# david8862/tf-keras-speech-commands

Measured on AMD Instinct MI355X. Metric: 1 s@16 kHz clips/sec train-step, simple_cnn bs4096, 1/2/4/8 MI355X; eval top-1, higher is better.
Workload: dtype f32; 1 GPU; configs[1]: simple_cnn train step = featurize(f32 1 s @16 kHz) + fwd + bwd + Adam, 36 logits (background + 35 words), batch 4096 per GPU; global_batch=4096, parallelism=dp1, gradient_exchange=none (one rank), rccl_ranks=0, library_build=546ca62dfe01

## Files before the change

### tf-keras-speech-commands_amd/csrc/kws_conv.h

```cpp
#pragma once
#include "kws_device.h"

namespace kws {

struct ConvGeom {
    int B, H, W, Ho, Wo;
    int stride, pt, pl;
    int KH, KW;
    int pmajor = 0;
};

enum { EPI_NONE = 0, EPI_RELU = 1, EPI_BIAS_RELU6 = 2, EPI_BIAS = 3, EPI_BIAS_RELU = 4,
       EPI_BN_RELU6 = 5,
       EPI_BNBWD_GATE6 = 6 };
enum { MODE_FWD = 0, MODE_DGRAD = 1 };

__host__ __device__ constexpr int stride16(int c) { return (c % 32 == 16) ? c : c + 16; }

template <int CR, int CO, int MODE, int EPI>
__global__ __launch_bounds__(256) void conv_gemm_kernel(const float *__restrict__ src, const float *__restrict__ wgt,
                                                         const float *__restrict__ bias, float *__restrict__ dst,
                                                         ConvGeom g)
{
    constexpr int KC = CR >= 32 ? 32 : CR;
// ... 570 lines not shown
        __syncthreads();
#pragma unroll
        for (int mt = 0; mt < MT; ++mt)
#pragma unroll
            for (int nw = 0; nw < NW; ++nw)
#pragma unroll
                for (int r = 0; r < 4; ++r) red[(16 * mt + 4 * lq + r) * COUT + 16 * (wave * NW + nw) + li] = acc[t][mt][nw][r];
        __syncthreads();
        if (nchunks > 0)
            for (int i = tid; i < CIN * COUT; i += 256) atomicAdd(dw + (long)(tap0 + t) * CIN * COUT + i, red[i]);
    }
}

template <int N>
__device__ __forceinline__ void load_vec(const float *__restrict__ p, float (&v)[N])
{
    if constexpr (N == 1) {
        v[0] = p[0];
    } else if constexpr (N == 2) {
        const float2 t = *reinterpret_cast<const float2 *>(p);
        v[0] = t.x; v[1] = t.y;
    } else {
#pragma unroll
        for (int i = 0; i < N / 4; ++i) {
            const float4 t = *reinterpret_cast<const float4 *>(p + 4 * i);
            v[4 * i] = t.x; v[4 * i + 1] = t.y; v[4 * i + 2] = t.z; v[4 * i + 3] = t.w;
        }
    }
}

template <int CIN, int COUT, int GPB>
__global__ __launch_bounds__(256) void conv_wgrad_direct_kernel(const float *__restrict__ x, const float *__restrict__ dz,
                                                                 float *__restrict__ dw, const float *__restrict__ zeros,
                                                                 ConvGeom g, int steps_per_wave)
{
    constexpr int CB = CIN >= 64 ? 64 : CIN;
    constexpr int CBLK = CIN / CB;
    constexpr int MT = CB / 16, NT = COUT / 16;
    static_assert(CIN % CB == 0 && CB % 16 == 0 && COUT % 16 == 0, "channel counts must be multiples of 16");
    extern __shared__ __attribute__((aligned(16))) float red[];

    const int lane = threadIdx.x & 63, wave = threadIdx.x >> 6, li = lane & 15, lq = lane >> 4;
    const long M = (long)g.B * g.Ho * g.Wo;
    const int HoWo = g.Ho * g.Wo;
    const int ngroups = g.KH * g.KW * CBLK, grp0 = blockIdx.y * GPB;
    const long step0 = ((long)blockIdx.x * 4 + wave) * steps_per_wave;

    int kh[GPB], kw[GPB], cb[GPB], toff[GPB];
    bool gok[GPB];
#pragma unroll
    for (int gi = 0; gi < GPB; ++gi) {
        const int grp = grp0 + gi, tap = grp / CBLK;
        gok[gi] = grp < ngroups;
        kh[gi] = tap / g.KW;
        kw[gi] = tap % g.KW;
        cb[gi] = (grp % CBLK) * CB;
        toff[gi] = (kh[gi] * g.W + kw[gi]) * CIN + cb[gi];
    }

    f32x4 acc[GPB][MT][NT];
#pragma unroll
    for (int gi = 0; gi < GPB; ++gi)
#pragma unroll
        for (int mt = 0; mt < MT; ++mt)
#pragma unroll
            for (int nt = 0; nt < NT; ++nt) acc[gi][mt][nt] = (f32x4){0.f, 0.f, 0.f, 0.f};

    long p = step0 * 4 + lq;
    int b = (int)(p / HoWo), rem = (int)(p % HoWo), oh = rem / g.Wo, ow = rem % g.Wo;
    auto load_frags = [&](float (&af)[GPB][MT], float (&bf)[NT]) {
        const bool pok = p < M;
        load_vec<NT>(pok ? dz + ((int)p * COUT + NT * li) : zeros + NT * li, bf);
        const int y0 = oh * g.stride - g.pt, x0 = ow * g.stride - g.pl;
// ... 982 lines not shown
```

### tf-keras-speech-commands_amd/csrc/kws_device.h

```cpp
#pragma once
#include <hip/hip_runtime.h>
#include <stdint.h>

namespace kws {

typedef float f32x4 __attribute__((ext_vector_type(4)));


__device__ __forceinline__ f32x4 mfma16(float a, float b, f32x4 c)
{
    return __builtin_amdgcn_mfma_f32_16x16x4f32(a, b, c, 0, 0, 0);
}

typedef __bf16 bf16x8 __attribute__((ext_vector_type(8)));
typedef __bf16 bf16x4 __attribute__((ext_vector_type(4)));
__device__ __forceinline__ f32x4 mfma_bf16(bf16x8 a, bf16x8 b, f32x4 c)
{
    return __builtin_amdgcn_mfma_f32_16x16x32_bf16(a, b, c, 0, 0, 0);
}
__device__ __forceinline__ f32x4 mfma_bf16x6(const bf16x8 (&a)[3], const bf16x8 (&b)[3], f32x4 c)
{
    c = mfma_bf16(a[1], b[1], c);
    c = mfma_bf16(a[2], b[0], c);
    c = mfma_bf16(a[0], b[2], c);
// ... 49 lines not shown
    return __int_as_float(__builtin_amdgcn_readlane(__float_as_int(v), 63));
}
#undef KWS_DPP_ADD

struct HeadFwdArgs {
    const float *b2;
    const int32_t *labels;
    const float *class_w;
    float *probs, *loss_i_out, *correct_i_out;
    float grad_scale;
    int ignore_index;
};

constexpr int kAccSlots = 8, kAccDoubles = kAccSlots * 2 * 128;
__device__ __forceinline__ void acc_add(double *__restrict__ acc, int C2, int i, double v)
{
    atomicAdd(acc + (blockIdx.x & (kAccSlots - 1)) * C2 + i, v);
}
__device__ __forceinline__ double acc_sum(const double *__restrict__ acc, int C2, int i)
{
    double v[kAccSlots];
#pragma unroll
    for (int j = 0; j < kAccSlots; ++j) v[j] = acc[j * C2 + i];
    double t = 0.0;
#pragma unroll
    for (int j = 0; j < kAccSlots; ++j) t += v[j];
    return t;
}
__device__ __forceinline__ void acc_clear(double *__restrict__ acc, int tid, int nthreads)
{
    for (int i = tid; i < kAccDoubles; i += nthreads) acc[i] = 0.0;
}

}
```

### tf-keras-speech-commands_amd/csrc/kws_layers.h

```cpp
#pragma once
#include "kws_device.h"

namespace kws {

constexpr float kBnEps = 1e-3f;
constexpr double kBnMomentum = 0.99;
constexpr float kCeEps = 1e-7f;
constexpr int kStatStride = 1024;

__device__ __forceinline__ double block_sum_partials(const double *__restrict__ partial, int which, int C, int c, int nblk,
                                                     double *sh )
{
    double s = 0.0;
    for (int b = threadIdx.x; b < nblk; b += 256) s += partial[((long)which * C + c) * kStatStride + b];
    sh[threadIdx.x] = s;
    __syncthreads();
    for (int o = 128; o > 0; o >>= 1) {
        if ((int)threadIdx.x < o) sh[threadIdx.x] += sh[threadIdx.x + o];
        __syncthreads();
    }
    s = sh[0];
    __syncthreads();
    return s;
}
// ... 449 lines not shown
    f32x4 d;
#pragma unroll
    for (int e = 0; e < 4; ++e) {
        const int c = c0 + e;
        const float xhat = (zv[e] - k.mean[c]) * k.inv[c];
        float v = gamma[c] * k.inv[c] * (gv[e] - k.k2[c] - xhat * k.k3[c]);
        if (RELU_IN) v = zv[e] > 0.f ? v : 0.f;
        d[e] = v;
    }
    bf16x4 h, m, l;
    split_bf16(d, h, m, l);
    reinterpret_cast<bf16x4 *>(out.p[0])[i4] = h;
    reinterpret_cast<bf16x4 *>(out.p[1])[i4] = m;
    reinterpret_cast<bf16x4 *>(out.p[2])[i4] = l;
}

struct BnAccBwd { const double *acc; double *acc_clear_set; long M; float *dgamma, *dbeta; };
__device__ __forceinline__ void bn_bwd_k_prologue(const BnAccBwd &a, const BnCoef &k, int C, float *kk)
{
    const int i = threadIdx.x;
    if (i < 2 * C) {
        const double t = acc_sum(a.acc, 2 * C, i);
        const float kv = (float)(t / (double)a.M);
        kk[i] = kv;
        if (blockIdx.x == 0) {
            if (i < C) { a.dbeta[i] = (float)t; k.k2[i] = kv; }
            else { a.dgamma[i - C] = (float)t; k.k3[i - C] = kv; }
        }
    }
    if (blockIdx.x == 0 && a.acc_clear_set) acc_clear(a.acc_clear_set, threadIdx.x, blockDim.x);
    __syncthreads();
}

template <bool RELU_IN>
__global__ __launch_bounds__(256) void bn_bwd_apply_routed_planes_kernel(const float *__restrict__ z, const float *__restrict__ gq,
                                                                          const unsigned char *__restrict__ arg, BnCoef k,
                                                                          const float *__restrict__ gamma, int B, int H, int W, int C,
                                                                          BnAccBwd a, Bf16PlanesOut out)
{
    __shared__ float kk[256];
    bn_bwd_k_prologue(a, k, C, kk);
    const int Hp = H / 2, Wp = W / 2, C4 = C / 4;
    const long total4 = (long)B * H * W * C4;
    for (long i4 = (long)blockIdx.x * 256 + threadIdx.x; i4 < total4; i4 += (long)gridDim.x * 256) {
        const int c0 = (int)(i4 % C4) * 4;
        const long pix = i4 / C4;
        const int p = (int)(pix % ((long)H * W)), b = (int)(pix / ((long)H * W)), y = p / W, x = p - y * W, ph = y >> 1, pw = x >> 1;
        const f32x4 zv = reinterpret_cast<const f32x4 *>(z)[i4];
        f32x4 gv = {0.f, 0.f, 0.f, 0.f};
        if (ph < Hp && pw < Wp) {
            const long q = (((long)b * Hp + ph) * Wp + pw) * C + c0;
            const f32x4 g4 = *reinterpret_cast<const f32x4 *>(gq + q);
            const unsigned a4 = *reinterpret_cast<const unsigned *>(arg + q), e = (unsigned)((y & 1) * 2 + (x & 1));
#pragma unroll
            for (int j = 0; j < 4; ++j) gv[j] = ((a4 >> (8 * j)) & 0xffu) == e ? g4[j] : 0.f;
        }
        f32x4 d;
#pragma unroll
        for (int j = 0; j < 4; ++j) {
            const int c = c0 + j;
            const float xhat = (zv[j] - k.mean[c]) * k.inv[c];
            float v = gamma[c] * k.inv[c] * (gv[j] - kk[c] - xhat * kk[C + c]);
            if (RELU_IN) v = zv[j] > 0.f ? v : 0.f;
            d[j] = v;
        }
        bf16x4 h, m, l;
        split_bf16(d, h, m, l);
        reinterpret_cast<bf16x4 *>(out.p[0])[i4] = h;
        reinterpret_cast<bf16x4 *>(out.p[1])[i4] = m;
        reinterpret_cast<bf16x4 *>(out.p[2])[i4] = l;
    }
}

template <bool RELU_IN>
__global__ __launch_bounds__(256) void bn_bwd_apply_acc_kernel(const float *__restrict__ z, float *__restrict__ gz, BnCoef k,
                                                                const float *__restrict__ gamma, long total4, int C, BnAccBwd a)
{
    __shared__ float kk[256];
    bn_bwd_k_prologue(a, k, C, kk);
    const int C4 = C / 4;
    for (long i4 = (long)blockIdx.x * 256 + threadIdx.x; i4 < total4; i4 += (long)gridDim.x * 256) {
        const int c0 = (int)(i4 % C4) * 4;
        const f32x4 zv = reinterpret_cast<const f32x4 *>(z)[i4], gv = reinterpret_cast<const f32x4 *>(gz)[i4];
        f32x4 d;
#pragma unroll
        for (int j = 0; j < 4; ++j) {
            const int c = c0 + j;
            const float xhat = (zv[j] - k.mean[c]) * k.inv[c];
            float v = gamma[c] * k.inv[c] * (gv[j] - kk[c] - xhat * kk[C + c]);
            if (RELU_IN) v = zv[j] > 0.f ? v : 0.f;
            d[j] = v;
        }
        reinterpret_cast<f32x4 *>(gz)[i4] = d;
    }
}

__global__ __launch_bounds__(256) void head_fwd_kernel(const float *__restrict__ d1, const float *__restrict__ w2,
                                                        const float *__restrict__ b2, const int32_t *__restrict__ labels,
                                                        const float *__restrict__ class_w, float *__restrict__ probs,
                                                        int32_t *__restrict__ argmax_out, float *__restrict__ loss_i,
                                                        float *__restrict__ correct_i, float *__restrict__ dlogits, int B,
                                                        int K, int C, float grad_scale, int ignore_index)
{
    extern __shared__ float hs[];
    float *xs = hs;
    float *lg = hs + 16 * K;
    const int b0 = blockIdx.x * 16;
    for (int i = threadIdx.x; i < 16 * K; i += 256) {
        const int s = i / K;
        xs[i] = (b0 + s < B) ? d1[(long)(b0 + s) * K + (i % K)] : 0.f;
    }
    __syncthreads();
    for (int i = threadIdx.x; i < 16 * C; i += 256) {
        const int s = i / C, c = i % C;
        float acc = 0.f;
        for (int k = 0; k < K; ++k) acc = fmaf(xs[s * K + k], w2[(long)k * C + c], acc);
        lg[i] = acc + b2[c];
    }
    __syncthreads();
    if (threadIdx.x < 16 && b0 + threadIdx.x < B) {
        const int s = threadIdx.x, b = b0 + s;
        float mx = lg[s * C];
        int am = 0;
        for (int c = 1; c < C; ++c)
            if (lg[s * C + c] > mx) { mx = lg[s * C + c]; am = c; }
        float sum = 0.f;
// ... 63 lines not shown
        if (omx > mx || (omx == mx && oam < am)) { mx = omx; am = oam; }
    }
    float sum = 0.f;
    for (int c = j; c < C; c += 16) { const float e = expf(lg[s * C + c] - mx); lg[s * C + c] = e; sum += e; }
#pragma unroll
    for (int o = 8; o > 0; o >>= 1) sum += __shfl_xor(sum, o, 16);
    const float rs = 1.f / sum;
    if (b >= B) return;
    if (argmax_out && j == 0) argmax_out[b] = am;
    if (probs)
        for (int c = j; c < C; c += 16) probs[(long)b * C + c] = lg[s * C + c] * rs;
    if (labels) {
        const int y = labels[b];
        const float py = lg[s * C + y] * rs;
        float loss, coef;
        if (class_w) {
            loss = -logf(py) * class_w[y];
            coef = class_w[y];
        } else {
            const float lo = kCeEps, hi = 1.f - kCeEps;
            loss = -logf(fminf(fmaxf(py, lo), hi));
            coef = (py >= lo && py <= hi) ? 1.f : 0.f;
        }
        if (ignore_index > 0 && y == ignore_index) { loss = 0.f; coef = 0.f; }
        if (j == 0) { loss_i[b] = loss; correct_i[b] = am == y ? 1.f : 0.f; }
        if (dlogits)
            for (int c = j; c < C; c += 16) dlogits[(long)b * C + c] = (lg[s * C + c] * rs - (c == y ? 1.f : 0.f)) * coef * grad_scale;
    }
}

__global__ __launch_bounds__(256) void loss_reduce_kernel(const float *__restrict__ loss_i, const float *__restrict__ correct_i,
                                                           int B, float *__restrict__ out)
{
    double s = 0.0, c = 0.0;
    for (int i = threadIdx.x; i < B; i += 256) { s += (double)loss_i[i]; c += (double)correct_i[i]; }
    __shared__ double sh[2][256];
    sh[0][threadIdx.x] = s;
    sh[1][threadIdx.x] = c;
    __syncthreads();
    for (int o = 128; o > 0; o >>= 1) {
        if (threadIdx.x < o) { sh[0][threadIdx.x] += sh[0][threadIdx.x + o]; sh[1][threadIdx.x] += sh[1][threadIdx.x + o]; }
        __syncthreads();
    }
    if (threadIdx.x == 0) { out[0] = (float)sh[0][0]; out[1] = (float)sh[1][0]; }
}

constexpr int kHeadBwdRows = 16;

template <bool RELU6_GATE>
__global__ __launch_bounds__(256) void head_bwd_kernel(const float *__restrict__ x, const float *__restrict__ w2,
                                                        const float *__restrict__ dlogits, float *__restrict__ dx,
                                                        float *__restrict__ dw2, float *__restrict__ db2, int B, int K, int C)
{
    extern __shared__ float hs[];
    float *xs = hs;
    float *ds = hs + kHeadBwdRows * K;
    const int b0 = blockIdx.x * kHeadBwdRows;
    for (int i = threadIdx.x; i < kHeadBwdRows * K; i += 256) xs[i] = (b0 + i / K < B) ? x[(long)(b0 + i / K) * K + (i % K)] : 0.f;
    for (int i = threadIdx.x; i < kHeadBwdRows * C; i += 256) ds[i] = (b0 + i / C < B) ? dlogits[(long)(b0 + i / C) * C + (i % C)] : 0.f;
    __syncthreads();
    for (int i = threadIdx.x; i < kHeadBwdRows * K; i += 256) {
        const int s = i / K, k = i % K;
        if (b0 + s >= B) continue;
        float acc = 0.f;
        for (int c = 0; c < C; ++c) acc = fmaf(ds[s * C + c], w2[(long)k * C + c], acc);
        if (RELU6_GATE) { const float xv = xs[i]; acc = (xv > 0.f && xv < 6.f) ? acc : 0.f; }
        dx[(long)(b0 + s) * K + k] = acc;
    }
    for (int i = threadIdx.x; i < K * C; i += 256) {
        const int k = i / C, c = i % C;
        float acc = 0.f;
        for (int s = 0; s < kHeadBwdRows; ++s) acc = fmaf(xs[s * K + k], ds[s * C + c], acc);
        if (dw2) atomicAdd(dw2 + i, acc);
    }
    for (int c = threadIdx.x; c < C; c += 256) {
        float acc = 0.f;
        for (int s = 0; s < kHeadBwdRows; ++s) acc += ds[s * C + c];
// ... 267 lines not shown
```

### tf-keras-speech-commands_amd/csrc/kws_model.hip

```cpp
#include <cstdlib>
#include <cstring>
#include <string>
#include <type_traits>
#include <vector>

#include "kws_common.h"
#include "kws_model_types.h"
#include "kws_conv.h"
#include "kws_layers.h"
#include "kws_layer1.h"
#include "kws_layer1_moments.h"
#include "kws_layer1_fast.h"
#include "kws_l1_conv2.h"
#include "kws_conv2_wgrad_fast.h"
#include "kws_lite.h"
#include "kws_lite_f16.h"
#include "kws_infer_fused.h"
#include "kws_conv_group.h"
#include "kws_dense_head.h"
#include "kws_cnn_plan.h"

using namespace kws;

namespace {
// ... 131 lines not shown
    KWS_LAUNCH("bn_infer_coef_all_kernel", bn_infer_coef_all_kernel, dim3(4), dim3(128), 0, s, a);
    return KWS_OK;
}

inline void stat_grid(long M, int C, int &nblk, int &rows)
{
    const int R = 256 / C;
    long want = (M + (long)R * 8 - 1) / ((long)R * 8);
    nblk = (int)std::min<long>(kMaxStatBlocks, std::max<long>(1, want));
    rows = (int)((M + nblk - 1) / nblk);
    nblk = (int)((M + rows - 1) / rows);
}

template <int CR, int CO, int MODE, int EPI>
int launch_gemm(const float *src, const float *w, const float *bias, float *dst, const ConvGeom &g, hipStream_t s)
{
    const long M = (long)g.B * g.Ho * g.Wo;
    static const std::string name = std::string("conv_gemm_fwd<") + std::to_string(CR) + "," +
                                    std::to_string(CO) + ">";
    KWS_LAUNCH(name.c_str(), (conv_gemm_kernel<CR, CO, MODE, EPI>), dim3(blocks_for(M, 64)), dim3(256), 0, s, src, w, bias, dst, g);
    return KWS_OK;
}

static int cu_count() { return device_cus(); }
template <typename K>
static int resident_blocks(K kernel, int threads, size_t smem)
{
    int nb = 0;
    if (hipOccupancyMaxActiveBlocksPerMultiprocessor(&nb, kernel, threads, smem) != hipSuccess || nb < 1) { (void)hipGetLastError(); nb = 1; }
    return nb;
}

template <int CIN, int COUT, int GPB>
int launch_wgrad(const float *x, const float *dz, float *dw, const ConvGeom &g, hipStream_t s, bool deterministic = false)
{
    const float *zp = zero_page();
    if (!zp) return fail(KWS_ERR_NOMEM, "cannot allocate the zero page on this device");
    constexpr int CB = CIN >= 64 ? 64 : CIN;
    constexpr size_t smem = (4 * 64 * 4 + 16 * COUT) * sizeof(float);
    const long M = (long)g.B * g.Ho * g.Wo;
    const int ngroups = g.KH * g.KW * (CIN / CB), gy = (ngroups + GPB - 1) / GPB;
    const long steps = (M + 3) / 4;
    static const int occ = resident_blocks(conv_wgrad_direct_kernel<CIN, COUT, GPB>, 256, smem);
    const long slots = deterministic ? 1 : std::max<long>(1, (long)cu_count() * occ / gy);
    const long gx_want = std::max<long>(1, std::min<long>(slots, (steps + 4 * 8 - 1) / (4 * 8)));
    const int spw = (int)((steps + 4 * gx_want - 1) / (4 * gx_want));
    const long gx = (steps + 4L * spw - 1) / (4L * spw);
    static const std::string name = "conv_wgrad<" + std::to_string(CIN) + "," + std::to_string(COUT) + ">";
    KWS_LAUNCH(name.c_str(), (conv_wgrad_direct_kernel<CIN, COUT, GPB>), dim3((unsigned)gx, (unsigned)gy), dim3(256), smem,
               s, x, dz, dw, zp, g, spw);
    return KWS_OK;
}

template <int CIN, int COUT, int TPB, bool DPRE = false, bool XBN = false>
int launch_wgrad_bf16(const float *x, const float *dz, float *dw, const ConvGeom &g, hipStream_t s, __bf16 *const *dz_planes = nullptr,
                      bool deterministic = false, const float *xbn = nullptr)
{
    if (TPB != 1 && g.KW != TPB) return fail(KWS_ERR_UNSUPPORTED, "split-precision weight gradient expects a kernel %d taps wide", TPB);
    const float *zp = zero_page();
    if (!zp) return fail(KWS_ERR_NOMEM, "cannot allocate the zero page on this device");
    constexpr size_t stage = (size_t)3 * 32 * 4 * (TPB * tr_row_words(CIN) + tr_row_words(COUT)), tile = (size_t)CIN * COUT * sizeof(float);
    constexpr size_t smem = stage > tile ? stage : tile;
    if (int rc = ensure_dynamic_lds(reinterpret_cast<const void *>(conv_wgrad_bf16_kernel<CIN, COUT, TPB, DPRE, XBN>), (int)smem)) return rc;
    static const int occ = resident_blocks(conv_wgrad_bf16_kernel<CIN, COUT, TPB, DPRE, XBN>, 256, smem);
    const long M = (long)g.B * g.Ho * g.Wo, nchunk = (M + 31) / 32;
    const int ngroups = g.KH * g.KW / TPB;
    long nranges = std::max<long>(8, ((long)cu_count() * occ / ngroups) / 8 * 8);
    nranges = std::min<long>(nranges, std::max<long>(8, (nchunk / 4 + 7) / 8 * 8));
    int cpb = (int)((nchunk + nranges - 1) / nranges);
    if (deterministic) { nranges = 8; cpb = (int)nchunk; }
    static const std::string name = "conv_wgrad_bf16<" + std::to_string(CIN) + "," + std::to_string(COUT) + ">";
    const Bf16Planes dpl{{DPRE ? dz_planes[0] : nullptr, DPRE ? dz_planes[1] : nullptr, DPRE ? dz_planes[2] : nullptr}};
    KWS_LAUNCH(name.c_str(), (conv_wgrad_bf16_kernel<CIN, COUT, TPB, DPRE, XBN>), dim3((unsigned)(nranges * ngroups)), dim3(256), smem, s, x, dz, dw,
               zp, g, cpb, (int)nranges, dpl, xbn);
    return KWS_OK;
}

template <int CR, int CO, int MW, int STRIDE>
int launch_dgrad_mw(const float *dz, const float *w, float *dx, const ConvGeom &g, const DgradClasses &cls, int ncls, long max_rows,
                     hipStream_t s)
{
    static const std::string name = "conv_dgrad<" + std::to_string(CR) + "," + std::to_string(CO) + ">";
    const float *zp = zero_page();
// ... 200 lines not shown
    g.B = B; g.H = H; g.W = W; g.Ho = H; g.Wo = W; g.stride = 1; g.pt = 0; g.pl = 0; g.KH = 1; g.KW = 1;
    return g;
}
static ConvGeom dense_geom(const CnnDims &d, int B)
{
    ConvGeom g;
    g.B = B; g.H = d.H4; g.W = d.W4; g.Ho = 1; g.Wo = 1; g.stride = 1; g.pt = 0; g.pl = 0; g.KH = d.H4; g.KW = d.W4;
    return g;
}

constexpr int kPrepSplitBlocks = 16, kPrepZeroBlocks = 16, kPrepBlocks = 3 * kPrepSplitBlocks + kPrepZeroBlocks;

struct CnnStep {
    const kws_model *m;
    const CnnDims &d;
    int B;
    const float *feat, *params;
    float *state, *grads;
    CnnWs &w;
    hipStream_t s;
    uint64_t dropout_seed;

    uint32_t slo() const { return (uint32_t)(dropout_seed & 0xFFFFFFFFu); }
    uint32_t shi() const { return (uint32_t)(dropout_seed >> 32); }
    float drop_rate() const { return dropout_seed != 0 ? 0.5f : 0.f; }
    BnCoef coef(int l) const { return coef_of(w.coef[l], kCh[l + 1]); }
    long pixels(int l) const { const CnnStage t = cnn_stage(d, l); return (long)B * t.Ho * t.Wo; }

    int bn_train_coefs(int l, int fused_stat_blocks = 0);
    int bn_act(int l, float rate, float *zm = nullptr, unsigned char *ag = nullptr);
    int bn_bwd_finalize(int l, int nblk);
    template <bool RELU> int bn_bwd_apply(int l);
    int colsum(const char *label, const float *x, long M, int C, float *dst);
    int dense_fwd(), dense_bias_grad(), dense_wgrad(hipStream_t on, bool det), dense_dgrad();
    int head_infer(float *probs, int32_t *argmax) { return run_head(m, B, params, w.d1, w.loss_i, w.correct_i, nullptr, nullptr, probs, argmax, nullptr, 0.f, nullptr, 0, s); }
    int head_train(const kws_train_args *a, float *stats);
};

struct CnnCtx : CnnStep {
    ModelRes *R;
    hipStream_t s2;
    const CnnPlan &P;
    OverlapHook *hook;
    const double *moments;
    const kws_train_args *a;
    float *probs;
    int32_t *argmax;
    unsigned fpar[4], bpar[4];
    bool bound6;
    int fused_bn3_blocks;

    BnAccFwd acc_in(int l, unsigned parity) const
    {
        return BnAccFwd{acc_set(R, 0, l, parity), acc_set(R, 0, l, parity + 1), pixels(l), params + m->o_g[l], params + m->o_b[l],
                        state + m->o_mm[l], state + m->o_mv[l], coef(l)};
    }
    BnAccBwd acc_out(int l) const { return BnAccBwd{acc_set(R, 1, l, bpar[l]), acc_set(R, 1, l, bpar[l] + 1), pixels(l), grads + m->o_g[l], grads + m->o_b[l]}; }

    int forward();
    int fwd_prepare(), fwd_layer1(), fwd_conv2(), fwd_conv3(), fwd_conv4(), fwd_dense();
    int backward();
    int bwd_head_dense(), bwd_layer4(), bwd_layer3(), bwd_layer2(), bwd_layer1();
    void bwd_arm(int ev) { arm_stop_event(R->ev[ev], s); }
    int bwd_fork(int ev);
    int bwd_reduce_pool(int l, int H, int W, int C, float *da, float rate, int nblk, int rows);
};

// ... 131 lines not shown
    const int C = kCh[l + 1];
    KWS_LAUNCH(prof_name("bn_bwd_finalize_kernel", l + 1), bn_bwd_finalize_kernel, dim3(C), dim3(64), 0, s, w.partial, nblk, pixels(l), C, params + m->o_g[l],
               grads + m->o_g[l], grads + m->o_b[l], coef(l));
    return KWS_OK;
}
template <bool RELU>
int CnnStep::bn_bwd_apply(int l)
{
    const int C = kCh[l + 1];
    const long total = pixels(l) * C;
    KWS_LAUNCH(prof_name("bn_bwd_apply_kernel", l + 1), bn_bwd_apply_kernel<RELU>, dim3(blocks_for(total, 256)), dim3(256), 0, s, w.z[l], w.gz[l], coef(l),
               params + m->o_g[l], total, C);
    return KWS_OK;
}

int CnnStep::colsum(const char *label, const float *x, long M, int C, float *dst)
{
    int nblk, rows;
    stat_grid(M, C, nblk, rows);
    KWS_LAUNCH(label, channel_stats_kernel, dim3(nblk), dim3(256), 0, s, x, M, C, rows, w.partial);
    KWS_LAUNCH("colsum_finalize_kernel", colsum_finalize_kernel, dim3(C), dim3(256), 0, s, w.partial, nblk, C, dst);
    return KWS_OK;
}
int CnnStep::head_train(const kws_train_args *a, float *stats)
{
    KWS_TRY(run_head(m, B, params, w.d1, w.loss_i, w.correct_i, a->labels, a->class_weights, a->probs, nullptr, w.dlogits, a->grad_scale / (float)B,
                     stats, a->ignore_index, s));
    if (a->forward_event) KWS_HIP_CHECK(hipEventRecord(static_cast<hipEvent_t>(a->forward_event), s));
    return KWS_OK;
}

int CnnStep::dense_fwd() { return launch_gemm<128, 128, MODE_FWD, EPI_BIAS_RELU6>(w.a[3], params + m->o_dk, params + m->o_db, w.d1, dense_geom(d, B), s); }
int CnnStep::dense_bias_grad() { return colsum("channel_stats_kernel.dense", w.dd1, B, 128, grads + m->o_db); }
int CnnStep::dense_wgrad(hipStream_t on, bool det) { return launch_wgrad<128, 128, 1>(w.a[3], w.dd1, grads + m->o_dk, dense_geom(d, B), on, det); }
int CnnStep::dense_dgrad() { return launch_dgrad<128, 128, 1>(w.dd1, params + m->o_dk, w.da4, dense_geom(d, B), s); }

int CnnCtx::fwd_conv2()
{
    const float *in = w.a[0], *kern = params + m->o_k[1];
    const unsigned nblk = (unsigned)std::min(B, kMaxStatBlocks);
    const Conv2Clip cc = conv2_clip(d, B);
    if (!P.training) {
        const BnCoef k2 = coef(1);
        if (P.bf16) {
            KWS_LAUNCH("conv_fwd_clip_pool_bf16<16,32>", (conv_fwd_clip_bf16_kernel<false, true>), dim3(nblk), dim3(256), cc.smb, s, in, kern, w.a[1], B,
                       d.H1, d.W1, w.partial, kStatStride, k2.scale, k2.shift);
            if (P.fused_tail) KWS_TRY(launch_fused_tail(m, B, params, w, probs, argmax, s));
        } else
            KWS_LAUNCH("conv_fwd_clip_pool<16,32>", (conv_fwd_clip_kernel<32, false, true>), dim3(nblk), dim3(256), cc.sm, s, in, kern, w.a[1], B,
                       d.H1, d.W1, w.partial, kStatStride, k2.scale, k2.shift);
        return KWS_OK;
    }
    if (P.l1_conv2) ;
    else if (P.bf16)
        KWS_LAUNCH("conv_fwd_clip_bf16<16,32>", (conv_fwd_clip_bf16_kernel<true>), dim3(nblk), dim3(256), cc.smb, s, in, kern, w.z[1], B, d.H1,
                   d.W1, w.partial, kStatStride, nullptr, nullptr, P.acc_fwd ? acc_set(R, 0, 1, fpar[1]) : nullptr);
    else
        KWS_LAUNCH("conv_fwd_clip<16,32>", (conv_fwd_clip_kernel<32, true>), dim3(nblk), dim3(256), cc.sm, s, in, kern, w.z[1], B, d.H1, d.W1,
                   w.partial, kStatStride);
    if (hook) KWS_TRY(hook->fire(9, s));
    if (!P.acc_fwd) KWS_TRY(bn_train_coefs(1, (int)nblk));
    if (!P.fuse_pool2) KWS_TRY(bn_act(1, 0.f, P.routed_g2 ? w.zmax2 : nullptr, P.routed_g2 ? w.arg2 : nullptr));
    return KWS_OK;
}

int CnnCtx::fwd_conv3()
{
// ... 106 lines not shown
        da.B = B; da.C = m->C; da.flat = d.flat;
        if (P.acc_bn4) {
            da.zmax4 = w.zmax4; da.coef4 = coef(3).scale; da.acc4 = acc_set(R, 1, 3, bpar[3]);
            da.drop_rate = drop_rate(); da.seed_lo = slo(); da.seed_hi = shi();
        }
        if (P.pool4_fused) {
            da.z4 = w.z[3]; da.a4w = w.a[3]; da.zmax4w = w.zmax4; da.arg4w = w.arg4; da.H3 = d.H3; da.W3 = d.W3;
            da.in4 = acc_in(3, R->acc_uses[0][3] - 1);
            da.drop_rate = drop_rate(); da.seed_lo = slo(); da.seed_hi = shi();
        }
        da.fw = HeadFwdArgs{params + m->o_hb, a->labels, a->class_weights, a->probs, w.loss_i, w.correct_i, a->grad_scale / (float)B, a->ignore_index};
        const size_t smem = sizeof(float) * (size_t)(16 * (d.flat + 8) + 2 * 16 * kDhKS + 16 * kDhCS + kDhK * kDhCS);
        if (int rc = ensure_dynamic_lds(reinterpret_cast<const void *>(dense_head_fused_kernel), (int)smem)) return rc;
        KWS_LAUNCH("dense_head_fused_kernel", dense_head_fused_kernel, dim3(blocks_for(B, 16)), dim3(kDhThreads), smem, s, da);
    } else if (P.fuse_head_fwd) {
        const HeadFwdArgs hf{params + m->o_hb, a->labels, a->class_weights, a->probs, w.loss_i, w.correct_i, a->grad_scale / (float)B, a->ignore_index};
        KWS_TRY(run_head_bwd(m, B, params, w.d1, nullptr, w.dd1, grads, true, s, grads + m->o_db, nullptr, nullptr, nullptr, false, &hf));
    } else
        KWS_TRY(run_head_bwd(m, B, params, w.d1, w.dlogits, w.dd1, grads, true, s, nullptr, w.loss_i, w.correct_i,
                             stats, P.det));
    const bool fork0_bound = stop_event_bound(fork0_ev);
    if (P.fuse_head_fwd) {
        if (a->forward_event) KWS_HIP_CHECK(hipEventRecord(static_cast<hipEvent_t>(a->forward_event), s));
        if (hook) KWS_TRY(hook->fire(1, s));
    }
    const bool hook_ev_here = hook && hook->wants(2) && hook->ev;
    if (hook) KWS_TRY(hook->fire(2, s, fork0_bound && hook_ev_here));
    if (hook_ev_here) {
        KWS_HIP_CHECK(hipStreamWaitEvent(s2, fork0_ev, 0));
    } else {
        if (!fork0_bound) KWS_HIP_CHECK(hipEventRecord(R->ev[0], s));
        KWS_HIP_CHECK(hipStreamWaitEvent(s2, R->ev[0], 0));
    }
    if (P.fuse_head_fwd && stats) KWS_LAUNCH("loss_reduce_kernel", loss_reduce_kernel, dim3(1), dim3(256), 0, s2, w.loss_i, w.correct_i, B, stats);
    KWS_TRY(dense_wgrad(s2, P.det));
    if (!P.fuse_head_fwd) KWS_TRY(dense_bias_grad());
    if (P.dense_fused) ;
    else if (P.bf16) KWS_TRY_NB(launch_bf16<128, 128, MODE_DGRAD, EPI_NONE>("conv_bf16_dgrad", w.dd1, w.wsp[2], nullptr, w.da4, dense_geom(d, B), s));
    else KWS_TRY(dense_dgrad());
    if (hook) KWS_TRY(hook->fire(3, s));
    return KWS_OK;
}

int CnnCtx::bwd_layer4()
{
    const int C = 128, H = d.H3, W = d.W3;
    const long M = pixels(3);
    const BnCoef k = coef(3);
    const float *gamma = params + m->o_g[3];
    const float rate = drop_rate();
    int nblk, rows;
    stat_grid((long)B * (H / 2) * (W / 2), C, nblk, rows);
    if (P.acc_bn4) ;
    else if (P.bf16)
        KWS_LAUNCH(prof_name("bn_bwd_reduce_pool_kernel", 4), bn_bwd_reduce_routed_full_kernel, dim3(nblk), dim3(256), 0, s, w.zmax4, w.arg4, w.da4, k,
                   w.gz[3], B, H, W, C, rows, w.partial, rate, slo(), shi());
    else KWS_TRY(bwd_reduce_pool(3, H, W, C, w.da4, rate, nblk, rows));
    if (!P.acc_bn4) KWS_TRY(bn_bwd_finalize(3, nblk));
    bwd_arm(3);
    const Bf16PlanesOut dzp{{w.dzp[0], w.dzp[1], w.dzp[2]}};
    if (P.acc_bn4)
        KWS_LAUNCH(prof_name("bn_bwd_apply_planes_kernel", 4), bn_bwd_apply_routed_planes_kernel<true>, dim3(std::min<unsigned>(1024u, blocks_for(M * C / 4, 256))),
                   dim3(256), 0, s, w.z[3], w.da4, w.arg4, k, gamma, B, H, W, C, acc_out(3), dzp);
    else if (P.bf16)
        KWS_LAUNCH(prof_name("bn_bwd_apply_planes_kernel", 4), bn_bwd_apply_planes_kernel<true>, dim3(blocks_for(M * C / 4, 256)), dim3(256), 0, s,
                   w.z[3], w.gz[3], k, gamma, M * C / 4, C, dzp);
    else KWS_TRY(bn_bwd_apply<true>(3));
    if (hook) KWS_TRY(hook->fire(4, s));
    KWS_TRY(bwd_fork(3));
    const float *in = w.a[2], *kern = params + m->o_k[3];
    float *dk = grads + m->o_k[3];
    const ConvGeom g = geom3x3(B, H, W, 1);
    if (P.bf16 && P.a3_on_load)
        KWS_TRY((launch_wgrad_bf16<64, 128, 1, true, true>(w.z[2], nullptr, dk, g, s2, w.dzp, P.det, coef(2).scale)));
    else if (P.bf16) KWS_TRY(launch_wgrad_bf16<64, 128, 1, true>(in, nullptr, dk, g, s2, w.dzp, P.det));
    else KWS_TRY(launch_wgrad<64, 128, 1>(in, w.gz[3], dk, g, s2, P.det));
    if (a->comm) KWS_TRY(comm_allreduce_early(a->comm, grads + m->o_k[3], m->P - m->o_k[3], s2));
    if (a->bucket_event) KWS_HIP_CHECK(hipEventRecord(static_cast<hipEvent_t>(a->bucket_event), s2));
    if (P.group) {
        fused_bn3_blocks = launch_group_dgrad4(m, B, w, s, P.acc_bn3 ? acc_set(R, 1, 2, bpar[2]) : nullptr);
        if (fused_bn3_blocks < 0) return fused_bn3_blocks;
    } else if (P.bf16 && blocks_for(M, 64) <= (unsigned)kStatStride) {
        const BnCoef k3 = coef(2);
        fused_bn3_blocks = launch_bf16<128, 64, MODE_DGRAD, EPI_BNBWD_GATE6>("conv_bf16_dgrad", nullptr, w.wsp[1], k3.scale, w.gz[2], g, s, w.partial,
                                                                             w.z[2], w.dzp);
        if (fused_bn3_blocks < 0) return fused_bn3_blocks;
    } else if (P.bf16)
        KWS_TRY_NB(launch_bf16<128, 64, MODE_DGRAD, EPI_NONE>("conv_bf16_dgrad", nullptr, w.wsp[1], nullptr, w.da[2], g, s, nullptr, nullptr, w.dzp));
    else KWS_TRY(launch_dgrad<128, 64, 1>(w.gz[3], kern, w.da[2], g, s));
    return KWS_OK;
}

int CnnCtx::bwd_layer3()
{
    const int C = 64, H = d.H3, W = d.W3;
    if (hook) KWS_TRY(hook->fire(5, s));
    const long M = pixels(2);
// ... 796 lines not shown
```

Measured before the change: 7.533 million clips/s.

## Fold loss reduction into dense wgrad grid and prefetch routed BN-backward loads

The separate single-block loss/accuracy reduction kernel is removed. Its work now runs in one extra block appended to the dense weight-gradient launch, which saves a kernel launch on the side stream. The routed BN-backward apply kernel gets a walking variant with 32-bit indexing. It advances pixel coordinates incrementally instead of dividing, and processes six units per thread. The first batch of loads is issued before the accumulator prologue so memory latency overlaps the reduction read. The extra block adds shared-memory assumptions to the wgrad kernel, and the walk path is guarded by a size check.

```diff
diff --git a/tf-keras-speech-commands_amd/csrc/kws_conv.h b/tf-keras-speech-commands_amd/csrc/kws_conv.h
--- a/tf-keras-speech-commands_amd/csrc/kws_conv.h
+++ b/tf-keras-speech-commands_amd/csrc/kws_conv.h
@@ -626,13 +626,18 @@
 template <int CIN, int COUT, int GPB>
 __global__ __launch_bounds__(256) void conv_wgrad_direct_kernel(const float *__restrict__ x, const float *__restrict__ dz,
                                                                  float *__restrict__ dw, const float *__restrict__ zeros,
-                                                                 ConvGeom g, int steps_per_wave)
+                                                                 ConvGeom g, int steps_per_wave, LossSumJob job)
 {
     constexpr int CB = CIN >= 64 ? 64 : CIN;
     constexpr int CBLK = CIN / CB;
     constexpr int MT = CB / 16, NT = COUT / 16;
     static_assert(CIN % CB == 0 && CB % 16 == 0 && COUT % 16 == 0, "channel counts must be multiples of 16");
     extern __shared__ __attribute__((aligned(16))) float red[];
+
+    if (job.out && blockIdx.x == gridDim.x - 1) {
+        if (blockIdx.y == 0) loss_sum_block(job.loss_i, job.correct_i, job.B, job.out, reinterpret_cast<double *>(red));
+        return;
+    }
 
     const int lane = threadIdx.x & 63, wave = threadIdx.x >> 6, li = lane & 15, lq = lane >> 4;
     const long M = (long)g.B * g.Ho * g.Wo;
diff --git a/tf-keras-speech-commands_amd/csrc/kws_device.h b/tf-keras-speech-commands_amd/csrc/kws_device.h
--- a/tf-keras-speech-commands_amd/csrc/kws_device.h
+++ b/tf-keras-speech-commands_amd/csrc/kws_device.h
@@ -105,4 +105,20 @@
     for (int i = tid; i < kAccDoubles; i += nthreads) acc[i] = 0.0;
 }
 
+struct LossSumJob { const float *loss_i, *correct_i; float *out; int B; };
+__device__ __forceinline__ void loss_sum_block(const float *__restrict__ loss_i, const float *__restrict__ correct_i, int B,
+                                               float *__restrict__ out, double *sh)
+{
+    double s = 0.0, c = 0.0;
+    for (int i = threadIdx.x; i < B; i += 256) { s += (double)loss_i[i]; c += (double)correct_i[i]; }
+    sh[threadIdx.x] = s;
+    sh[256 + threadIdx.x] = c;
+    __syncthreads();
+    for (int o = 128; o > 0; o >>= 1) {
+        if (threadIdx.x < o) { sh[threadIdx.x] += sh[threadIdx.x + o]; sh[256 + threadIdx.x] += sh[256 + threadIdx.x + o]; }
+        __syncthreads();
+    }
+    if (threadIdx.x == 0) { out[0] = (float)sh[0]; out[1] = (float)sh[256]; }
 }
+
+}
diff --git a/tf-keras-speech-commands_amd/csrc/kws_layers.h b/tf-keras-speech-commands_amd/csrc/kws_layers.h
--- a/tf-keras-speech-commands_amd/csrc/kws_layers.h
+++ b/tf-keras-speech-commands_amd/csrc/kws_layers.h
@@ -505,43 +505,129 @@
     __syncthreads();
 }
 
+struct BnBwdCh { float mean[4], inv[4], gamma[4], k2[4], k3[4]; };
+__device__ __forceinline__ BnBwdCh bn_bwd_channels(const BnCoef &k, const float *__restrict__ gamma, const float *kk, int C, int c0)
+{
+    BnBwdCh o;
+#pragma unroll
+    for (int j = 0; j < 4; ++j) {
+        o.mean[j] = k.mean[c0 + j]; o.inv[j] = k.inv[c0 + j]; o.gamma[j] = gamma[c0 + j];
+        o.k2[j] = kk[c0 + j]; o.k3[j] = kk[C + c0 + j];
+    }
+    return o;
+}
 template <bool RELU_IN>
+__device__ __forceinline__ f32x4 bn_bwd_unit(const f32x4 zv, const f32x4 gv, const BnBwdCh &o)
+{
+    f32x4 d;
+#pragma unroll
+    for (int j = 0; j < 4; ++j) {
+        const float xhat = (zv[j] - o.mean[j]) * o.inv[j];
+        float v = o.gamma[j] * o.inv[j] * (gv[j] - o.k2[j] - xhat * o.k3[j]);
+        if (RELU_IN) v = zv[j] > 0.f ? v : 0.f;
+        d[j] = v;
+    }
+    return d;
+}
+constexpr int kBnRoutedUnits = 6;
+inline bool bn_bwd_walk_ok(long total4, int C, unsigned blocks, int units)
+{
+    return C % 4 == 0 && 256 % (C / 4) == 0 && (total4 + (long)units * blocks * 256) * 16 < (1L << 31);
+}
+__device__ __forceinline__ f32x4 load_f32x4_at(const float *__restrict__ p, unsigned byte_off)
+{
+    return *reinterpret_cast<const f32x4 *>(reinterpret_cast<const char *>(p) + byte_off);
+}
+struct BnWalk { unsigned b, p, db, dp, HW, W, Hp, Wp; };
+
+template <int N> struct BnRoutedRegs { f32x4 zv[N], g4[N]; unsigned a4[N], e[N]; };
+template <int N>
+__device__ __forceinline__ void bn_routed_load(const float *__restrict__ z, const float *__restrict__ gq, const unsigned char *__restrict__ arg,
+                                               unsigned C, unsigned c0, unsigned i4, unsigned stride, BnWalk &wk, BnRoutedRegs<N> &r)
+{
+#pragma unroll
+    for (int u = 0; u < N; ++u) {
+        const unsigned y = wk.p / wk.W, x = wk.p - y * wk.W;
+        const bool win = (y >> 1) < wk.Hp && (x >> 1) < wk.Wp;
+        const unsigned q = win ? ((wk.b * wk.Hp + (y >> 1)) * wk.Wp + (x >> 1)) * C + c0 : c0;
+        r.e[u] = win ? (y & 1) * 2 + (x & 1) : 0x100u;
+        r.zv[u] = load_f32x4_at(z, (i4 + u * stride) * 16u);
+        r.g4[u] = load_f32x4_at(gq, q * 4u);
+        r.a4[u] = *reinterpret_cast<const unsigned *>(arg + q);
+        wk.p += wk.dp; wk.b += wk.db;
+        if (wk.p >= wk.HW) { wk.p -= wk.HW; ++wk.b; }
+    }
+}
+template <bool RELU_IN, int N>
+__device__ __forceinline__ void bn_routed_finish(const Bf16PlanesOut &out, const BnBwdCh &ch, unsigned i4, unsigned stride, const BnRoutedRegs<N> &r)
+{
+#pragma unroll
+    for (int u = 0; u < N; ++u) {
+        f32x4 gv;
+#pragma unroll
+        for (int j = 0; j < 4; ++j) gv[j] = ((r.a4[u] >> (8 * j)) & 0xffu) == r.e[u] ? r.g4[u][j] : 0.f;
+        bf16x4 h, m, l;
+        split_bf16(bn_bwd_unit<RELU_IN>(r.zv[u], gv, ch), h, m, l);
+        const unsigned off = (i4 + u * stride) * 8u;
+        *reinterpret_cast<bf16x4 *>(reinterpret_cast<char *>(out.p[0]) + off) = h;
+        *reinterpret_cast<bf16x4 *>(reinterpret_cast<char *>(out.p[1]) + off) = m;
+        *reinterpret_cast<bf16x4 *>(reinterpret_cast<char *>(out.p[2]) + off) = l;
+    }
+}
+
+template <bool RELU_IN, bool WALK>
 __global__ __launch_bounds__(256) void bn_bwd_apply_routed_planes_kernel(const float *__restrict__ z, const float *__restrict__ gq,
                                                                           const unsigned char *__restrict__ arg, BnCoef k,
                                                                           const float *__restrict__ gamma, int B, int H, int W, int C,
                                                                           BnAccBwd a, Bf16PlanesOut out)
 {
     __shared__ float kk[256];
-    bn_bwd_k_prologue(a, k, C, kk);
     const int Hp = H / 2, Wp = W / 2, C4 = C / 4;
-    const long total4 = (long)B * H * W * C4;
-    for (long i4 = (long)blockIdx.x * 256 + threadIdx.x; i4 < total4; i4 += (long)gridDim.x * 256) {
-        const int c0 = (int)(i4 % C4) * 4;
-        const long pix = i4 / C4;
-        const int p = (int)(pix % ((long)H * W)), b = (int)(pix / ((long)H * W)), y = p / W, x = p - y * W, ph = y >> 1, pw = x >> 1;
-        const f32x4 zv = reinterpret_cast<const f32x4 *>(z)[i4];
-        f32x4 gv = {0.f, 0.f, 0.f, 0.f};
-        if (ph < Hp && pw < Wp) {
-            const long q = (((long)b * Hp + ph) * Wp + pw) * C + c0;
-            const f32x4 g4 = *reinterpret_cast<const f32x4 *>(gq + q);
-            const unsigned a4 = *reinterpret_cast<const unsigned *>(arg + q), e = (unsigned)((y & 1) * 2 + (x & 1));
-#pragma unroll
-            for (int j = 0; j < 4; ++j) gv[j] = ((a4 >> (8 * j)) & 0xffu) == e ? g4[j] : 0.f;
-        }
-        f32x4 d;
-#pragma unroll
-        for (int j = 0; j < 4; ++j) {
-            const int c = c0 + j;
-            const float xhat = (zv[j] - k.mean[c]) * k.inv[c];
-            float v = gamma[c] * k.inv[c] * (gv[j] - kk[c] - xhat * kk[C + c]);
-            if (RELU_IN) v = zv[j] > 0.f ? v : 0.f;
-            d[j] = v;
-        }
-        bf16x4 h, m, l;
-        split_bf16(d, h, m, l);
-        reinterpret_cast<bf16x4 *>(out.p[0])[i4] = h;
-        reinterpret_cast<bf16x4 *>(out.p[1])[i4] = m;
-        reinterpret_cast<bf16x4 *>(out.p[2])[i4] = l;
+    if constexpr (WALK) {
+        constexpr int kU = kBnRoutedUnits;
+        const unsigned total4 = (unsigned)B * H * W * C4, stride = gridDim.x * 256u, HW = (unsigned)(H * W);
+        const unsigned c0 = threadIdx.x % (unsigned)C4 * 4u;
+        unsigned i4 = blockIdx.x * 256u + threadIdx.x;
+        const unsigned pix = i4 / C4, pstep = stride / C4;
+        BnWalk wk{pix / HW, pix % HW, pstep / HW, pstep % HW, HW, (unsigned)W, (unsigned)Hp, (unsigned)Wp};
+        const bool ahead = i4 + (kU - 1) * stride < total4;
+        BnRoutedRegs<kU> r0;
+        if (ahead) bn_routed_load<kU>(z, gq, arg, C, c0, i4, stride, wk, r0);
+        bn_bwd_k_prologue(a, k, C, kk);
+        const BnBwdCh ch = bn_bwd_channels(k, gamma, kk, C, (int)c0);
+        if (ahead) { bn_routed_finish<RELU_IN, kU>(out, ch, i4, stride, r0); i4 += kU * stride; }
+        for (; i4 + (kU - 1) * stride < total4; i4 += kU * stride) {
+            BnRoutedRegs<kU> r;
+            bn_routed_load<kU>(z, gq, arg, C, c0, i4, stride, wk, r);
+            bn_routed_finish<RELU_IN, kU>(out, ch, i4, stride, r);
+        }
+        for (; i4 < total4; i4 += stride) {
+            BnRoutedRegs<1> r;
+            bn_routed_load<1>(z, gq, arg, C, c0, i4, stride, wk, r);
+            bn_routed_finish<RELU_IN, 1>(out, ch, i4, stride, r);
+        }
+    } else {
+        bn_bwd_k_prologue(a, k, C, kk);
+        const long total4 = (long)B * H * W * C4;
+        for (long i4 = (long)blockIdx.x * 256 + threadIdx.x; i4 < total4; i4 += (long)gridDim.x * 256) {
+            const int c0 = (int)(i4 % C4) * 4;
+            const long pix = i4 / C4;
+            const int p = (int)(pix % ((long)H * W)), b = (int)(pix / ((long)H * W)), y = p / W, x = p - y * W, ph = y >> 1, pw = x >> 1;
+            const f32x4 zv = reinterpret_cast<const f32x4 *>(z)[i4];
+            f32x4 gv = {0.f, 0.f, 0.f, 0.f};
+            if (ph < Hp && pw < Wp) {
+                const long q = (((long)b * Hp + ph) * Wp + pw) * C + c0;
+                const f32x4 g4 = *reinterpret_cast<const f32x4 *>(gq + q);
+                const unsigned a4 = *reinterpret_cast<const unsigned *>(arg + q), e = (unsigned)((y & 1) * 2 + (x & 1));
+#pragma unroll
+                for (int j = 0; j < 4; ++j) gv[j] = ((a4 >> (8 * j)) & 0xffu) == e ? g4[j] : 0.f;
+            }
+            bf16x4 h, m, l;
+            split_bf16(bn_bwd_unit<RELU_IN>(zv, gv, bn_bwd_channels(k, gamma, kk, C, c0)), h, m, l);
+            reinterpret_cast<bf16x4 *>(out.p[0])[i4] = h;
+            reinterpret_cast<bf16x4 *>(out.p[1])[i4] = m;
+            reinterpret_cast<bf16x4 *>(out.p[2])[i4] = l;
+        }
     }
 }
 
@@ -553,18 +639,8 @@
     bn_bwd_k_prologue(a, k, C, kk);
     const int C4 = C / 4;
     for (long i4 = (long)blockIdx.x * 256 + threadIdx.x; i4 < total4; i4 += (long)gridDim.x * 256) {
-        const int c0 = (int)(i4 % C4) * 4;
         const f32x4 zv = reinterpret_cast<const f32x4 *>(z)[i4], gv = reinterpret_cast<const f32x4 *>(gz)[i4];
-        f32x4 d;
-#pragma unroll
-        for (int j = 0; j < 4; ++j) {
-            const int c = c0 + j;
-            const float xhat = (zv[j] - k.mean[c]) * k.inv[c];
-            float v = gamma[c] * k.inv[c] * (gv[j] - kk[c] - xhat * kk[C + c]);
-            if (RELU_IN) v = zv[j] > 0.f ? v : 0.f;
-            d[j] = v;
-        }
-        reinterpret_cast<f32x4 *>(gz)[i4] = d;
+        reinterpret_cast<f32x4 *>(gz)[i4] = bn_bwd_unit<RELU_IN>(zv, gv, bn_bwd_channels(k, gamma, kk, C, (int)(i4 % C4) * 4));
     }
 }
 
@@ -694,17 +770,8 @@
 __global__ __launch_bounds__(256) void loss_reduce_kernel(const float *__restrict__ loss_i, const float *__restrict__ correct_i,
                                                            int B, float *__restrict__ out)
 {
-    double s = 0.0, c = 0.0;
-    for (int i = threadIdx.x; i < B; i += 256) { s += (double)loss_i[i]; c += (double)correct_i[i]; }
-    __shared__ double sh[2][256];
-    sh[0][threadIdx.x] = s;
-    sh[1][threadIdx.x] = c;
-    __syncthreads();
-    for (int o = 128; o > 0; o >>= 1) {
-        if (threadIdx.x < o) { sh[0][threadIdx.x] += sh[0][threadIdx.x + o]; sh[1][threadIdx.x] += sh[1][threadIdx.x + o]; }
-        __syncthreads();
-    }
-    if (threadIdx.x == 0) { out[0] = (float)sh[0][0]; out[1] = (float)sh[1][0]; }
+    __shared__ double sh[2 * 256];
+    loss_sum_block(loss_i, correct_i, B, out, sh);
 }
 
 constexpr int kHeadBwdRows = 16;
diff --git a/tf-keras-speech-commands_amd/csrc/kws_model.hip b/tf-keras-speech-commands_amd/csrc/kws_model.hip
--- a/tf-keras-speech-commands_amd/csrc/kws_model.hip
+++ b/tf-keras-speech-commands_amd/csrc/kws_model.hip
@@ -187,7 +187,8 @@
 }
 
 template <int CIN, int COUT, int GPB>
-int launch_wgrad(const float *x, const float *dz, float *dw, const ConvGeom &g, hipStream_t s, bool deterministic = false)
+int launch_wgrad(const float *x, const float *dz, float *dw, const ConvGeom &g, hipStream_t s, bool deterministic = false,
+                 const LossSumJob *job = nullptr)
 {
     const float *zp = zero_page();
     if (!zp) return fail(KWS_ERR_NOMEM, "cannot allocate the zero page on this device");
@@ -202,8 +203,8 @@
     const int spw = (int)((steps + 4 * gx_want - 1) / (4 * gx_want));
     const long gx = (steps + 4L * spw - 1) / (4L * spw);
     static const std::string name = "conv_wgrad<" + std::to_string(CIN) + "," + std::to_string(COUT) + ">";
-    KWS_LAUNCH(name.c_str(), (conv_wgrad_direct_kernel<CIN, COUT, GPB>), dim3((unsigned)gx, (unsigned)gy), dim3(256), smem,
-               s, x, dz, dw, zp, g, spw);
+    KWS_LAUNCH(name.c_str(), (conv_wgrad_direct_kernel<CIN, COUT, GPB>), dim3((unsigned)gx + (job ? 1u : 0u), (unsigned)gy), dim3(256), smem,
+               s, x, dz, dw, zp, g, spw, job ? *job : LossSumJob{});
     return KWS_OK;
 }
 
@@ -470,7 +471,7 @@
     int bn_bwd_finalize(int l, int nblk);
     template <bool RELU> int bn_bwd_apply(int l);
     int colsum(const char *label, const float *x, long M, int C, float *dst);
-    int dense_fwd(), dense_bias_grad(), dense_wgrad(hipStream_t on, bool det), dense_dgrad();
+    int dense_fwd(), dense_bias_grad(), dense_wgrad(hipStream_t on, bool det, const LossSumJob *job = nullptr), dense_dgrad();
     int head_infer(float *probs, int32_t *argmax) { return run_head(m, B, params, w.d1, w.loss_i, w.correct_i, nullptr, nullptr, probs, argmax, nullptr, 0.f, nullptr, 0, s); }
     int head_train(const kws_train_args *a, float *stats);
 };
@@ -668,7 +669,10 @@
 
 int CnnStep::dense_fwd() { return launch_gemm<128, 128, MODE_FWD, EPI_BIAS_RELU6>(w.a[3], params + m->o_dk, params + m->o_db, w.d1, dense_geom(d, B), s); }
 int CnnStep::dense_bias_grad() { return colsum("channel_stats_kernel.dense", w.dd1, B, 128, grads + m->o_db); }
-int CnnStep::dense_wgrad(hipStream_t on, bool det) { return launch_wgrad<128, 128, 1>(w.a[3], w.dd1, grads + m->o_dk, dense_geom(d, B), on, det); }
+int CnnStep::dense_wgrad(hipStream_t on, bool det, const LossSumJob *job)
+{
+    return launch_wgrad<128, 128, 1>(w.a[3], w.dd1, grads + m->o_dk, dense_geom(d, B), on, det, job);
+}
 int CnnStep::dense_dgrad() { return launch_dgrad<128, 128, 1>(w.dd1, params + m->o_dk, w.da4, dense_geom(d, B), s); }
 
 int CnnCtx::fwd_conv2()
@@ -841,8 +845,8 @@
         if (!fork0_bound) KWS_HIP_CHECK(hipEventRecord(R->ev[0], s));
         KWS_HIP_CHECK(hipStreamWaitEvent(s2, R->ev[0], 0));
     }
-    if (P.fuse_head_fwd && stats) KWS_LAUNCH("loss_reduce_kernel", loss_reduce_kernel, dim3(1), dim3(256), 0, s2, w.loss_i, w.correct_i, B, stats);
-    KWS_TRY(dense_wgrad(s2, P.det));
+    const LossSumJob sums{w.loss_i, w.correct_i, stats, B};
+    KWS_TRY(dense_wgrad(s2, P.det, P.fuse_head_fwd && stats ? &sums : nullptr));
     if (!P.fuse_head_fwd) KWS_TRY(dense_bias_grad());
     if (P.dense_fused) ;
     else if (P.bf16) KWS_TRY_NB(launch_bf16<128, 128, MODE_DGRAD, EPI_NONE>("conv_bf16_dgrad", w.dd1, w.wsp[2], nullptr, w.da4, dense_geom(d, B), s));
@@ -868,10 +872,15 @@
     if (!P.acc_bn4) KWS_TRY(bn_bwd_finalize(3, nblk));
     bwd_arm(3);
     const Bf16PlanesOut dzp{{w.dzp[0], w.dzp[1], w.dzp[2]}};
-    if (P.acc_bn4)
-        KWS_LAUNCH(prof_name("bn_bwd_apply_planes_kernel", 4), bn_bwd_apply_routed_planes_kernel<true>, dim3(std::min<unsigned>(1024u, blocks_for(M * C / 4, 256))),
-                   dim3(256), 0, s, w.z[3], w.da4, w.arg4, k, gamma, B, H, W, C, acc_out(3), dzp);
-    else if (P.bf16)
+    if (P.acc_bn4) {
+        const unsigned nb = std::min<unsigned>(1024u, blocks_for(M * C / 4, 256));
+        if (bn_bwd_walk_ok(M * C / 4, C, nb, kBnRoutedUnits))
+            KWS_LAUNCH(prof_name("bn_bwd_apply_planes_kernel", 4), (bn_bwd_apply_routed_planes_kernel<true, true>), dim3(nb), dim3(256), 0, s, w.z[3], w.da4,
+                       w.arg4, k, gamma, B, H, W, C, acc_out(3), dzp);
+        else
+            KWS_LAUNCH(prof_name("bn_bwd_apply_planes_kernel", 4), (bn_bwd_apply_routed_planes_kernel<true, false>), dim3(nb), dim3(256), 0, s, w.z[3], w.da4,
+                       w.arg4, k, gamma, B, H, W, C, acc_out(3), dzp);
+    } else if (P.bf16)
         KWS_LAUNCH(prof_name("bn_bwd_apply_planes_kernel", 4), bn_bwd_apply_planes_kernel<true>, dim3(blocks_for(M * C / 4, 256)), dim3(256), 0, s,
                    w.z[3], w.gz[3], k, gamma, M * C / 4, C, dzp);
     else KWS_TRY(bn_bwd_apply<true>(3));
```

New measurement: 7.645 million clips/s (median of 6 runs). 1.5% higher.
